# GaetanBenoitDev/metaMDBG

Hardware: AMD Instinct MI355X
Metric: Gbp/s through minimizer+k-min-mer step; bit-exact k-min-mer table vs ref (higher is better)
Workload: dtype u64

## Files before the change

### metamdbg_amd/csrc/scan.hip

```cpp
#include "common.hpp"
#include "complexity_dev.hpp"
#include "murmur.hpp"
#include "objects.hpp"
#include "prefilter.hpp"
#include "scan_plan.hpp"
#include "segments_dev.hpp"

#include <fcntl.h>
#include <sys/file.h>
#include <sys/stat.h>
#include <unistd.h>

#include <algorithm>
#include <cerrno>
#include <cmath>
#include <cstdlib>
#include <memory>
#include <mutex>
#include <string>
#include <thread>
#include <type_traits>

namespace mdbg {

// ... 497 lines not shown
                uint32_t *dst = Q->orig + cb + o;
                const uint32_t w0 = tile_base_now + lane * 32u;
#pragma unroll
                for (int half = 0; half < 2; half++) {
                    uint32_t m = half ? (uint32_t)(d >> 32) : (uint32_t)d;
                    const uint32_t wb = w0 + 16u * half;
                    while (m) {
                        *dst++ = wb + (((uint32_t)__ffs((int)m) - 1u) >> 1);
                        m &= m - 1u;
                    }
                }
            }
            wave_lds_sync();
            if (lane == 0 && cb) { atomicOr(&S[0], carry); if (HAS_N && icarry) atomicOr(&SI[0], icarry); }
            if (c) {
                unsigned dst = 2u * (cb + o), w = dst >> 5, sh = dst & 31u;
                uint32_t yl = (uint32_t)y, yh = (uint32_t)(y >> 32);
                uint32_t p0 = yl << sh;
                uint32_t p1 = sh ? ((yl >> (32u - sh)) | (yh << sh)) : yh;
                uint32_t p2 = sh ? (yh >> (32u - sh)) : 0u;
                atomicOr(&S[w], p0);
                if (p1) atomicOr(&S[w + 1], p1);
                if (p2) atomicOr(&S[w + 2], p2);
                if (HAS_N) {
                    uint32_t ic = HPC ? compress_bits(iv, d) : (iv & (nvalid == 32 ? 0xFFFFFFFFu : ((1u << nvalid) - 1u)));
                    if (ic) {
                        unsigned di = cb + o, wq = di >> 5, sq = di & 31u;
                        atomicOr(&SI[wq], ic << sq);
                        if (sq && (ic >> (32u - sq))) atomicOr(&SI[wq + 1], ic >> (32u - sq));
                    }
                }
            }
            wave_lds_sync();

            const unsigned tot = cb + C;
            const unsigned nk = tot > K ? tot - K : 0u;
            const uint32_t hp_base = hp_total - cb;
            const uint32_t tile_base = t * TILE_WORDS * 32u;
            for (unsigned j0 = 0; j0 < nk; j0 += 64 * SCAN_PP) {
                const unsigned left = nk - j0;
                const unsigned pp = left >= 64u * SCAN_PP ? (unsigned)SCAN_PP : (left + 63u) / 64u;
                KmerTrip<HPC, HAS_QUAL, HAS_N> trip{a, S, SI, Q, K, kmask, kbits, comp_mask, lane, nk, hp_base, cb, tile_base, cap0, cap, r};
                if (pp == (unsigned)SCAN_PP && left >= 64u * SCAN_PP && hp_base + j0 >= a.trim) {
                    nout = trip.template run<SCAN_PP, true>(j0, nout);
                } else {
#if SCAN_PP <= 4
                    switch (pp) {
                        case 1: nout = trip.template run<1, false>(j0, nout); break;
                        case 2: nout = trip.template run<2, false>(j0, nout); break;
                        case 3: nout = trip.template run<3, false>(j0, nout); break;
                        default: nout = trip.template run<4, false>(j0, nout); break;
                    }
#else
                    if (pp <= 2) nout = trip.template run<2, false>(j0, nout);
                    else if (pp <= 4) nout = trip.template run<4, false>(j0, nout);
                    else nout = trip.template run<SCAN_PP, false>(j0, nout);
#endif
                }
            }

            const unsigned cbn = tot < K ? tot : K;
            const uint32_t cmask = (cbn >= 16) ? 0xFFFFFFFFu : ((1u << (2 * cbn)) - 1u);
            carry = cbn ? stream_extract(S, tot - cbn, cmask) : 0u;
            if (HAS_N) icarry = cbn ? istream_extract(SI, tot - cbn, (1u << cbn) - 1u) : 0u;
            uint32_t my_orig = 0;
            if (HAS_QUAL && HPC) { if (lane < cbn) my_orig = Q->orig[tot - cbn + lane]; }
            cb = cbn;
            hp_total += C;
            wave_lds_sync();
            if (HAS_QUAL && HPC) { if (lane < cbn) Q->orig[lane] = my_orig; }
        }

        if (a.trim == 0u && hp_total >= K) {
            if (HAS_QUAL && HPC) wave_lds_sync();
            const uint32_t e = carry & kmask;
            const uint32_t rev = e ^ comp_mask, fwd = digit_reverse(e, K);
            const uint32_t d = fwd < rev ? 0u : 1u, v = d ? rev : fwd;
            bool s1 = kmer_hash32(v) < a.threshold;
            if (HAS_N) s1 = s1 && icarry == 0u;
            if (s1 && a.n_rep) s1 = !rep_contains(a.rep, a.n_rep, v);
            if (s1) {
                if (lane == 0 && nout < cap) {
                    const uint32_t p = hp_total - K;
                    a.out_min[cap0 + nout] = v;
                    a.out_pos[cap0 + nout] = p;
                    a.out_dir[cap0 + nout] = (uint8_t)d;
                    if (HAS_QUAL) {
                        const uint32_t os = HPC ? Q->orig[0] : p;
                        const uint32_t oe = a.q_last ? (HPC ? Q->orig[K - 1] : p + K - 1u) + 1u : L;
                        if (a.inline_minq) {
                            const uint8_t *qq = a.qual + a.qual_off[r];
                            uint8_t mq = 255;
                            for (uint32_t bq = os; bq < oe; bq++) { uint8_t q = (uint8_t)(qq[bq] - 33); if (q < mq) mq = q; }
                            a.out_mqual[cap0 + nout] = mq;
                        } else {
                            a.out_os[cap0 + nout] = os;
                            a.out_oe[cap0 + nout] = oe;
                        }
                    }
                }
                nout++;
            }
        }

        uint8_t flags = 0;
        if (a.apply_filters && L >= 66) {
            if (complexity_suspect(wave_sum_u64(cx_bound), complexity_windows(L))) flags |= READ_SUSPECT;
        }
        if (lane == 0) {
            a.out_count[r] = nout;
            a.out_flags[r] = flags;
        }
    }
}

constexpr int FAST_BLOCK = 256;
constexpr int FAST_WAVES = FAST_BLOCK / 64;
constexpr unsigned RING_BASES = 16384;
constexpr unsigned DEFER_BLOCKS = 3;
constexpr unsigned SPAN = 32;
constexpr unsigned BLOCK_POS = 64 * SPAN;
constexpr bool DUAL_CHAIN = true;
constexpr int STAGE_CAP = 384;

struct SpanState {
    uint32_t fwd;
    uint32_t bits;
};

template <bool APPROX, bool K15 = false>
__device__ __forceinline__ void span_step(SpanState &st, uint32_t T, bool first, uint32_t kmask, uint32_t comp_mask, unsigned top_shift,
                                          unsigned K, uint64_t threshold, uint32_t cand_limit, uint32_t Tprev = 0u) {
    const uint32_t rev = (T ^ comp_mask) & kmask;
    if (K15) st.fwd = first ? digit_reverse(T & kmask, K) : (__builtin_amdgcn_alignbit(st.fwd, Tprev, 30) & kmask);
    else st.fwd = first ? digit_reverse(T & kmask, K) : (((st.fwd << 2) | ((T >> top_shift) & 3u)) & kmask);
    const uint32_t val = st.fwd < rev ? st.fwd : rev;
    if (APPROX) {
        const uint32_t s1 = kmer_hash32_hi_merged(val);
        asm("v_cmp_lt_u32 vcc, %1, %2\n\tv_addc_co_u32 %0, vcc, %0, %0, vcc" : "+v"(st.bits) : "v"(s1), "s"(cand_limit) : "vcc");
    } else {
        const uint64_t h = kmer_hash32(val);
        asm("v_cmp_lt_u64 vcc, %1, %2\n\tv_addc_co_u32 %0, vcc, %0, %0, vcc" : "+v"(st.bits) : "v"(h), "s"(threshold) : "vcc");
    }
}

__device__ __forceinline__ uint32_t ring_window(const uint32_t *S, unsigned p, unsigned wmask) {
    const unsigned b = 2u * p, w = (b >> 5) & wmask, sh = b & 31u;
    return __builtin_amdgcn_alignbit(S[(w + 1) & wmask], S[w], sh);
}

constexpr int HIST_TILES = 8;

constexpr unsigned PF_RING_BASES = 8192;
constexpr unsigned PF_DEFER_BLOCKS = 1;
constexpr int PF_STAGE_CAP = 176;
constexpr unsigned PF_LIST_CAP = 224;
template <int PFW> struct FastGeometry {
    static constexpr bool PF = PFW > 0;
    static constexpr int WAVES = PF ? PFW : FAST_WAVES, BLOCK = 64 * WAVES, STAGE = PF ? PF_STAGE_CAP : STAGE_CAP;
    static constexpr unsigned RING = PF ? PF_RING_BASES : RING_BASES, DEFER = PF ? PF_DEFER_BLOCKS : DEFER_BLOCKS;
    static constexpr unsigned RING_WORDS = RING / 16, RING_WMASK = RING_WORDS - 1;
    static constexpr size_t PF_LDS = PREFILTER_BYTES + 2 * HPC_LUT_SIZE + REP_FILTER_BITS / 8 + 16 +
                                     (size_t)WAVES * (RING / 4 + STAGE * 8 + PF_LIST_CAP * 2 + 64 * 4);
};
static_assert(FastGeometry<16>::PF_LDS + 28672 <= 163840, "16 waves fit beside the 28 KB the benchmark's other batch asks for");

template <bool HPC, bool QUAL, bool APPROX, int PFW = 0, bool SEG = false>
__global__ __launch_bounds__(FastGeometry<PFW>::BLOCK, PFW ? PFW / 4 : 5) void scan_fast_kernel(ScanArgs a) {
    using Geo = FastGeometry<PFW>;
    constexpr bool PF = Geo::PF;
    static_assert(!PF || (HPC && !QUAL && APPROX), "the bitmap holds the keys of compressed reads; its candidates are confirmed like APPROX ones");
    static_assert(Geo::DEFER * BLOCK_POS + 2 * BLOCK_POS + 17 <= Geo::RING, "deferred blocks + live bases fit the ring");
    __shared__ uint8_t lds_stage_q[QUAL ? Geo::WAVES : 1][QUAL ? Geo::STAGE : 1];
    __shared__ uint16_t lds_hist_o[(QUAL && HPC) ? Geo::WAVES * HIST_TILES * 64 : 1];
    __shared__ uint32_t lds_hist_c[(QUAL && HPC) ? Geo::WAVES : 1][(QUAL && HPC) ? HIST_TILES : 1];
    __shared__ alignas(16) uint32_t lds_ring[Geo::WAVES][Geo::RING_WORDS];
    __shared__ uint2 lds_stage[Geo::WAVES][Geo::STAGE];
    __shared__ alignas(16) uint8_t lds_lut[HPC ? 2 * HPC_LUT_SIZE : 16];
    const uint8_t *lds_lut_b = lds_lut, *lds_lut_n = lds_lut + (HPC ? HPC_LUT_SIZE : 0);
    __shared__ alignas(16) uint32_t lds_rep_filter[REP_FILTER_BITS / 32];
    if (HPC) hpc_lut_to_lds(lds_lut, threadIdx.x, Geo::BLOCK);
    static_assert((Geo::WAVES * Geo::RING_WORDS) % (4 * Geo::BLOCK) == 0 && (REP_FILTER_BITS / 32) % 4 == 0, "cleared as uint4");
#pragma unroll
    for (unsigned i = 0; i < Geo::WAVES * Geo::RING_WORDS / 4u; i += Geo::BLOCK) reinterpret_cast<uint4 *>(&lds_ring[0][0])[i + threadIdx.x] = make_uint4(0u, 0u, 0u, 0u);
    if (threadIdx.x < REP_FILTER_BITS / 128u) reinterpret_cast<uint4 *>(lds_rep_filter)[threadIdx.x] = make_uint4(0u, 0u, 0u, 0u);
    const uint8_t *pf_map = nullptr;
    uint16_t *pf_list_all = nullptr;
    uint32_t *pf_surv_all = nullptr, *pf_next = nullptr;
    if constexpr (PF) {
        __shared__ alignas(16) uint32_t lds_pf_map[PREFILTER_BYTES / 4];
        __shared__ uint16_t lds_pf_list[Geo::WAVES][PF_LIST_CAP];
        __shared__ uint32_t lds_pf_surv[Geo::WAVES][64];
        __shared__ uint32_t lds_pf_next;
        for (unsigned i = threadIdx.x; i < PREFILTER_BYTES / 16u; i += Geo::BLOCK)
            reinterpret_cast<uint4 *>(lds_pf_map)[i] = reinterpret_cast<const uint4 *>(a.pf_bits)[i];
        if (threadIdx.x == 0) lds_pf_next = 0u;
        pf_map = reinterpret_cast<const uint8_t *>(lds_pf_map);
        pf_list_all = &lds_pf_list[0][0]; pf_surv_all = &lds_pf_surv[0][0]; pf_next = &lds_pf_next;
    }
    __syncthreads();
    for (unsigned i = threadIdx.x; i < a.n_rep; i += Geo::BLOCK) {
        const uint32_t b = rep_filter_bit(a.rep[i]);
        atomicOr(&lds_rep_filter[b >> 5], 1u << (b & 31u));
    }
    __syncthreads();
    if (a.wave_priority == 1u) __builtin_amdgcn_s_setprio(1);
    else if (a.wave_priority == 2u) __builtin_amdgcn_s_setprio(2);
    else if (a.wave_priority >= 3u) __builtin_amdgcn_s_setprio(3);
    const unsigned lane = threadIdx.x & 63u;
    const unsigned wv = (unsigned)__builtin_amdgcn_readfirstlane((int)(threadIdx.x >> 6));
    uint32_t *S = lds_ring[wv];
    uint2 *stage = lds_stage[wv];
    uint8_t *stage_q = lds_stage_q[QUAL ? wv : 0];
    uint16_t *hist_o = lds_hist_o + ((QUAL && HPC) ? wv * HIST_TILES * 64 : 0);
    uint32_t *hist_c = lds_hist_c[(QUAL && HPC) ? wv : 0];
    const unsigned K = a.K;
    const uint32_t kmask = (K >= 16) ? 0xFFFFFFFFu : ((1u << (2 * K)) - 1u);
    const uint32_t comp_mask = 0xAAAAAAAAu & kmask;
    const unsigned top_shift = 2u * K - 2u;
    const uint64_t threshold = a.threshold;
    const uint64_t cand_limit64 = (threshold >> 32) + 3ull + (uint64_t)a.cand_slack;
    const uint32_t cand_limit = cand_limit64 > 0xFFFFFFFFull ? 0xFFFFFFFFu : (uint32_t)cand_limit64;
    const uint64_t guard_limit64 = 68ull + (uint64_t)a.guard_slack;
    const uint32_t guard_limit = guard_limit64 > 0xFFFFFFFFull ? 0xFFFFFFFFu : (uint32_t)guard_limit64;
    const bool unguarded = HPC && K == 15u && a.guard_slack == 0u;

    const uint32_t wave_global = blockIdx.x * Geo::WAVES + wv;
    const uint32_t n_waves = gridDim.x * Geo::WAVES;
    uint16_t *pf_list = PF ? pf_list_all + wv * PF_LIST_CAP : nullptr;
    uint32_t *pf_surv = PF ? pf_surv_all + wv * 64u : nullptr;
    const uint32_t pf_shift = a.pf_shift;
    const uint4 *const pf_table = PF ? a.pf_table : nullptr;
    const uint32_t pf_table_shift = a.pf_table_shift;
    constexpr uint32_t NO_READ = 0xFFFFFFFFu;
    const uint64_t chunk0 = (uint64_t)blockIdx.x * a.pf_chunk;
    const uint32_t chunk_n = PF ? (chunk0 >= a.n_reads ? 0u : (uint32_t)(a.n_reads - chunk0 < a.pf_chunk ? a.n_reads - chunk0 : a.pf_chunk)) : 0u;
    unsigned long long *const pf_counter = PF ? a.pf_counter : nullptr;
    uint32_t run_next = 0, run_end = 0, run_region = 0;
    auto take_read = [&]() -> uint32_t {
        if (pf_counter) {
            if (run_next == run_end) {
                uint32_t lo = 0, hi = 0;
                if (lane == 0) {
                    const unsigned long long s0 = __hip_atomic_fetch_add(pf_counter, (unsigned long long)a.pf_grab, __ATOMIC_RELAXED, __HIP_MEMORY_SCOPE_AGENT);
                    lo = (uint32_t)s0; hi = (uint32_t)(s0 >> 32);
                }
                lo = (uint32_t)__builtin_amdgcn_readfirstlane((int)lo); hi = (uint32_t)__builtin_amdgcn_readfirstlane((int)hi);
                if (hi || lo >= a.n_reads) return NO_READ;
                run_next = lo;
                run_end = a.n_reads - lo < a.pf_grab ? a.n_reads : lo + a.pf_grab;
                run_region = (lo / a.pf_grab) & (a.n_regions - 1u);
            }
            return run_next++;
        }
        uint32_t k = 0;
        if (lane == 0) k = atomicAdd(pf_next, 1u);
        k = (uint32_t)__builtin_amdgcn_readfirstlane((int)k);
        return k < chunk_n ? (uint32_t)chunk0 + k : NO_READ;
    };
    for (uint32_t r = PF ? take_read() : wave_global; PF ? r != NO_READ : r < a.n_reads; r = PF ? take_read() : r + n_waves) {
        if constexpr (PF && !SEG) { if (a.pf_len_split && a.len[r] >= a.pf_len_split) continue; }
        if (!SEG && a.skip && a.skip[r]) {
            if (a.cursor && lane == 0) { a.out_begin[r] = 0; a.out_count[r] = 0; a.out_flags[r] = 0; }
            continue;
        }
        SegView view{};
        if constexpr (SEG) {
            view = a.views[r];
            if (view.flags & SEG_DEAD) {
                if (lane == 0) { a.out_begin[r] = 0; a.out_count[r] = 0; a.out_flags[r] = 0; a.view_cx[r] = 0ull; }
                continue;
            }
        }
        const uint32_t rd = SEG ? view.read : r;
        const bool seg_inner = SEG && !(view.flags & SEG_FIRST);
        const uint32_t L = SEG ? view.raw_len : a.len[r];
        const uint64_t w_base = a.word_off[rd] + (SEG ? (uint64_t)view.tile0 * TILE_WORDS : 0ull);
        const uint64_t *rw = a.words + w_base;
        const uint32_t trim_first = seg_inner ? 0u : a.trim;
        const uint32_t nwords = (L + 31u) / 32u;
        const uint32_t ntiles = (nwords + TILE_WORDS - 1) / TILE_WORDS;
        const bool bump = a.cursor != nullptr;
        const uint64_t cap0 = bump ? 0ull : a.cap_off[r];
        const uint32_t cap = bump ? 0u : (uint32_t)(a.cap_off[r + 1] - cap0);
        uint32_t t_done = 0;
        uint32_t fill = 0;
        bool outgrown = false;

        auto orig_of = [&](uint32_t j, bool at_end) -> uint32_t {
            if (at_end && j >= fill) return L;
            uint32_t tt = t_done - 1u;
            const uint32_t t_low = t_done > (uint32_t)HIST_TILES ? t_done - (uint32_t)HIST_TILES : 0u;
            while (tt > t_low && hist_c[tt % HIST_TILES] > j) tt--;
            const uint32_t c0 = hist_c[tt % HIST_TILES];
            if (c0 > j) return 0xFFFFFFFFu;
            const uint32_t rel = j - c0;
            const uint16_t *o = hist_o + (tt % HIST_TILES) * 64u;
            uint32_t lo = 0;
#pragma unroll
            for (uint32_t st = 16; st >= 1; st >>= 2) {
                const uint32_t o1 = o[lo + st], o2 = o[lo + 2 * st], o3 = o[lo + 3 * st];
                lo += st * ((o1 <= rel ? 1u : 0u) + (o2 <= rel ? 1u : 0u) + (o3 <= rel ? 1u : 0u));
            }
            uint32_t k = rel - o[lo];
            const uint32_t wi = tt * TILE_WORDS + lo;
            const uint64_t x = rw[wi];
            const uint32_t pl = (wi || seg_inner) ? (uint32_t)(rw[(int64_t)wi - 1] >> 62) : (((uint32_t)x & 3u) ^ 1u);
            const int rem = (int)L - (int)(wi * 32u);
            const unsigned nvalid = rem >= 32 ? 32u : (unsigned)rem;
            const uint64_t vspread = nvalid == 32 ? M5 : (((1ull << (2 * nvalid)) - 1ull) & M5);
            const uint64_t diff = x ^ ((x << 2) | (uint64_t)pl);
            uint64_t m = (diff | (diff >> 1)) & vspread;
            uint32_t pos = 0;
#pragma unroll
            for (int sh = 32; sh >= 2; sh >>= 1) {
                const uint32_t c = (uint32_t)__popcll(m & ((1ull << sh) - 1ull));
                if (k >= c) { k -= c; m >>= sh; pos += (uint32_t)sh; }
            }
            return wi * 32u + (pos >> 1);
        };
        const uint8_t *qq = QUAL ? a.qual + a.qual_off[rd] + (SEG ? (uint64_t)view.tile0 * SEG_TILE_BASES : 0ull) : nullptr;
        auto min_quality = [&](uint32_t j, bool &known) -> uint8_t {
            uint32_t os = j, oe = j + K;
            if (HPC) {
                os = orig_of(j, false);
                const uint32_t last = orig_of(j + K - a.q_last, true);
                if (os == 0xFFFFFFFFu || last == 0xFFFFFFFFu) { known = false; return 0; }
                oe = last + a.q_last;
            }
            uint8_t mq = 255;
            for (uint32_t b0 = os; b0 < oe; b0 += 16) {
                uint64_t w[2];
                __builtin_memcpy(w, qq + b0, 16);
                const uint32_t nb = oe - b0 < 16u ? oe - b0 : 16u;
#pragma unroll
                for (unsigned b = 0; b < 16; b++) {
                    const uint8_t q = (uint8_t)((uint8_t)(w[b >> 3] >> (8 * (b & 7))) - 33);
                    if (b < nb && q < mq) mq = q;
                }
            }
            return mq;
        };

        bool lost = false;
        uint32_t n_false = 0;
        uint32_t n_staged_at_outgrowth = 0;
        uint32_t done = 0;
        uint32_t nout = 0;
        uint32_t flushed = 0;
        uint32_t n_mat = 0;
        uint32_t zero_from = 0;
        uint32_t prev_last = seg_inner ? (uint32_t)(rw[-1] >> 62) : 0u;
        static_assert((uint64_t)CX_Q_MAX * ((1ull << 24) / 16u) < (1ull << 32), "the 32-bit sum of a read below 2^24 bases");
        uint32_t cx_acc = 0;
        uint64_t cx_total = 0;
        const bool cx_long = L >= (1u << 24);
        uint64_t prev_word = seg_inner ? rw[-1] : 0ull;
        const uint32_t cx_nW = complexity_windows(SEG ? a.len[rd] : L);
        const uint32_t cx_tiles = SEG ? ((view.flags & SEG_LAST) ? ntiles : a.seg_tiles) : ntiles;
        const uint32_t cx_t0 = SEG ? view.tile0 : 0u;

        auto materialise = [&]() {
            const uint32_t pend = nout - n_mat;
            if (pend == 0u) return;
            if (outgrown) { n_mat = nout; return; }
            const uint32_t base = n_mat - flushed;
            for (uint32_t i = lane; i < pend; i += 64) {
                const uint32_t j = stage[base + i].y;
                const uint32_t e = ring_window(S, j, Geo::RING_WMASK) & kmask;
                const uint32_t rev = e ^ comp_mask, fw = digit_reverse(e, K);
                const uint32_t d = fw < rev ? 0u : 1u;
                if (QUAL) { bool known = true; stage_q[base + i] = min_quality(j, known); if (!known) lost = true; }
                stage[base + i] = make_uint2(d ? rev : fw, (j << 1) | d);
            }
            n_mat = nout;
            wave_lds_sync();
        };
        auto release_ring = [&](uint32_t upto) {
            const unsigned zb = zero_from >> 4, nz = (upto - zero_from) >> 4;
            for (unsigned i = lane; i < nz; i += 64) S[(zb + i) & Geo::RING_WMASK] = 0;
            zero_from = upto;
        };

        auto emit = [&](uint32_t bits, unsigned P, uint32_t npos_limit) {
            if constexpr (!PF) {
                if (P < 32u) bits &= (1u << P) - 1u;
                const uint32_t first_j = lane * P;
                if (first_j >= npos_limit) bits = 0;
                else if (first_j + P > npos_limit) bits &= ~((1u << (first_j + P - npos_limit)) - 1u);
                if (done == 0u && lane == 0u && trim_first) bits &= ~(1u << (P - 1u));
            }
            if (__ballot(bits != 0u) == 0ull) return;
            if (a.n_rep) {
                uint32_t b2 = bits;
                while (b2) {
                    const unsigned bit = 31u - (unsigned)__clz((int)b2);
                    b2 &= ~(1u << bit);
                    const unsigned u = P - 1u - bit;
                    const uint32_t e = ring_window(S, done + lane * P + u, Geo::RING_WMASK) & kmask;
                    const uint32_t rev = e ^ comp_mask, fw = digit_reverse(e, K);
                    const uint32_t v = fw < rev ? fw : rev, fb = rep_filter_bit(v);
                    if (((lds_rep_filter[fb >> 5] >> (fb & 31u)) & 1u) && rep_contains(a.rep, a.n_rep, v)) bits &= ~(1u << bit);
                }
            }
            const unsigned cnt = (unsigned)__popc(bits);
            const unsigned incl = wave_inclusive_sum_dpp(cnt);
            const unsigned total = (unsigned)__builtin_amdgcn_readlane((int)incl, 63);
            if (total == 0u) return;
            if (bump) {
                if (outgrown || nout + total > (unsigned)Geo::STAGE) {
                    if (!outgrown) { materialise(); n_staged_at_outgrowth = nout; }
                    if (APPROX && !PF) {
                        uint32_t bad = 0;
                        while (bits) {
                            const unsigned bit = 31u - (unsigned)__clz((int)bits);
                            bits &= ~(1u << bit);
                            const uint32_t e = ring_window(S, done + lane * P + (P - 1u - bit), Geo::RING_WMASK) & kmask;
                            const uint32_t rev = e ^ comp_mask, fw = digit_reverse(e, K);
                            if (!(kmer_hash32(fw < rev ? fw : rev) < threshold)) bad++;
                        }
                        n_false += (uint32_t)wave_sum_u64(bad);
                    }
                    outgrown = true; nout += total; return;
                }
            } else if (nout - flushed + total > (unsigned)Geo::STAGE) {
                materialise();
                const uint32_t ns = nout - flushed;
                for (uint32_t i = lane; i < ns; i += 64) {
                    const uint32_t idx = flushed + i;
                    if (idx < cap) {
                        const uint2 e = stage[i];
                        a.out_min[cap0 + idx] = e.x; a.out_pos[cap0 + idx] = e.y >> 1; a.out_dir[cap0 + idx] = (uint8_t)(e.y & 1u);
                        if (QUAL) a.out_mqual[cap0 + idx] = stage_q[i];
                    }
                }
                flushed = nout;
                wave_lds_sync();
            }
            if (total <= (unsigned)Geo::STAGE) {
                uint32_t at = nout - flushed + incl - cnt;
                while (bits) {
                    const unsigned bit = 31u - (unsigned)__clz((int)bits);
                    bits &= ~(1u << bit);
                    stage[at++].y = done + lane * P + (P - 1u - bit);
                }
                wave_lds_sync();
            } else {
                uint32_t at = nout + incl - cnt;
                while (bits) {
                    const unsigned bit = 31u - (unsigned)__clz((int)bits);
                    bits &= ~(1u << bit);
                    const unsigned u = P - 1u - bit;
                    const uint32_t j = done + lane * P + u;
                    const uint32_t e = ring_window(S, j, Geo::RING_WMASK) & kmask;
                    const uint32_t rev = e ^ comp_mask, fw = digit_reverse(e, K);
                    const uint32_t d = fw < rev ? 0u : 1u;
                    if (at < cap) {
                        a.out_min[cap0 + at] = d ? rev : fw; a.out_pos[cap0 + at] = j; a.out_dir[cap0 + at] = (uint8_t)d;
                        if (QUAL) { bool known = true; a.out_mqual[cap0 + at] = min_quality(j, known); if (!known) lost = true; }
                    }
                    at++;
                }
                flushed = nout + total;
                n_mat = nout + total;
            }
            nout += total;
        };

        auto pf_probe = [&](uint32_t v, uint32_t &b) {
            const uint32_t h = v * 0x9E3779B1u;
            const uint32_t byte = pf_map[h >> (pf_shift + 3u)];
            b = (b << 1) | ((byte >> ((h >> pf_shift) & 7u)) & 1u);
        };
        auto confirm = [&](uint32_t bits, unsigned P, uint32_t npos_limit) -> uint32_t {
            if (P < 32u) bits &= (1u << P) - 1u;
            {
                const uint32_t first_j = lane * P;
                if (first_j >= npos_limit) bits = 0;
                else if (first_j + P > npos_limit) bits &= ~((1u << (first_j + P - npos_limit)) - 1u);
                if (done == 0u && lane == 0u && trim_first) bits &= ~(1u << (P - 1u));
            }
            uint32_t kept = 0u;
            unsigned cnt = (unsigned)__popc(bits);
            unsigned incl = wave_inclusive_sum_dpp(cnt);
            unsigned total = (unsigned)__builtin_amdgcn_readlane((int)incl, 63);
            while (total != 0u) {
                pf_surv[lane] = 0u;
                unsigned at = incl - cnt;
                while (bits && at < PF_LIST_CAP) {
                    const unsigned bit = 31u - (unsigned)__clz((int)bits);
                    bits &= ~(1u << bit);
                    pf_list[at++] = (uint16_t)((lane << 5) | bit);
                }
                const unsigned n = total < PF_LIST_CAP ? total : PF_LIST_CAP;
                wave_lds_sync();
                auto listed_key = [&](uint32_t q) -> uint32_t {
                    const uint32_t e = ring_window(S, done + (q >> 5) * P + (P - 1u - (q & 31u)), Geo::RING_WMASK) & kmask;
                    const uint32_t rev = e ^ comp_mask, fw = digit_reverse(e, K);
                    return fw < rev ? fw : rev;
                };
                if (pf_table != nullptr) {
                    constexpr unsigned ROUNDS = (PF_LIST_CAP + 63u) / 64u;
                    uint32_t lh[ROUNDS];
                    uint4 lw[ROUNDS];
#pragma unroll
                    for (unsigned k = 0; k < ROUNDS; k++) {
                        lh[k] = 0u; lw[k] = make_uint4(0u, 0u, 0u, 0u);
                        if (64u * k < n) {
                            const unsigned i = lane + 64u * k;
                            if (i < n) {
                                lh[k] = confirm_hash(listed_key(pf_list[i]));
                                lw[k] = pf_table[lh[k] >> pf_table_shift];
                            }
                        }
                    }
                    uint32_t ask = 0u;
#pragma unroll
                    for (unsigned k = 0; k < ROUNDS; k++) {
                        if (64u * k < n) {
                            const uint32_t verdict = confirm_verdict(lw[k].x, lw[k].y, lw[k].z, lw[k].w, lh[k]);
                            if (verdict == CONFIRM_YES) { const uint32_t q = pf_list[lane + 64u * k]; atomicOr(&pf_surv[q >> 5], 1u << (q & 31u)); }
                            if (verdict == CONFIRM_ASK) ask |= 1u << k;
                        }
                    }
                    if (__ballot(ask != 0u) != 0ull) {
#pragma nounroll
                        for (unsigned k = 0; k < ROUNDS; k++) {
                            if ((ask >> k) & 1u) {
                                const uint32_t q = pf_list[lane + 64u * k];
                                if (kmer_hash32(listed_key(q)) < threshold) atomicOr(&pf_surv[q >> 5], 1u << (q & 31u));
                            }
                        }
                    }
                } else {
                    for (unsigned i = lane; i < n; i += 64u) {
                        const uint32_t q = pf_list[i];
                        if (kmer_hash32(listed_key(q)) < threshold) atomicOr(&pf_surv[q >> 5], 1u << (q & 31u));
                    }
                }
                wave_lds_sync();
                kept |= pf_surv[lane];
                if (total <= PF_LIST_CAP) break;
                wave_lds_sync();
                cnt = (unsigned)__popc(bits);
                incl = wave_inclusive_sum_dpp(cnt);
                total -= PF_LIST_CAP;
            }
            return kept;
        };

        auto guarded_redo = [&](unsigned P) -> uint32_t {
            SpanState rs{0u, 0u};
#pragma nounroll
            for (unsigned u = 0; u < P; u++)
                span_step<APPROX>(rs, ring_window(S, done + lane * P + u, Geo::RING_WMASK), u == 0u, kmask, comp_mask, top_shift, K, threshold, cand_limit);
            return rs.bits;
        };

        auto aligned_block = [&](auto sp_tag) {
            constexpr int SP = decltype(sp_tag)::value;
            constexpr unsigned WPL = (unsigned)SP / 16u;
            const unsigned wb = ((done >> 4) + WPL * lane) & Geo::RING_WMASK;
            const uint32_t W0 = S[wb], W1 = S[(wb + 1) & Geo::RING_WMASK], W2 = SP > 16 ? S[(wb + 2) & Geo::RING_WMASK] : 0u;
            SpanState st{0u, 0u};
            auto walk = [&](auto k15_tag, auto guard_tag) {
                constexpr bool K15 = decltype(k15_tag)::value;
                constexpr bool GUARD = APPROX && decltype(guard_tag)::value;
                if (SP == 32 && DUAL_CHAIN) {
                    uint32_t fa = 0u, fb = 0u, ba = 0u, bb = 0u, pa = 0u, pb = 0u;
                    uint32_t g = 0xFFFFFFFFu;
#pragma unroll
                    for (int u = 0; u < 16; u++) {
                        const uint32_t Ta = u == 0 ? W0 : __builtin_amdgcn_alignbit(W1, W0, 2 * u);
                        const uint32_t Tb = u == 0 ? W1 : __builtin_amdgcn_alignbit(W2, W1, 2 * u);
                        const uint32_t reva = (Ta ^ comp_mask) & kmask, revb = (Tb ^ comp_mask) & kmask;
                        if (u == 0) { fa = digit_reverse(Ta & kmask, K); fb = digit_reverse(Tb & kmask, K); }
                        else if (K15) { fa = __builtin_amdgcn_alignbit(fa, pa, 30) & kmask; fb = __builtin_amdgcn_alignbit(fb, pb, 30) & kmask; }
                        else { fa = ((fa << 2) | ((Ta >> top_shift) & 3u)) & kmask; fb = ((fb << 2) | ((Tb >> top_shift) & 3u)) & kmask; }
                        const uint32_t va = fa < reva ? fa : reva, vb = fb < revb ? fb : revb;
                        if (PF) {
                            pf_probe(va, ba); pf_probe(vb, bb);
                        } else if (APPROX) {
                            uint32_t ra, rb;
                            kmer_hash32_hi_shared_x2<GUARD>(va, vb, ra, rb, g);
                            asm("v_cmp_lt_u32 vcc, %1, %2\n\tv_addc_co_u32 %0, vcc, %0, %0, vcc" : "+v"(ba) : "v"(ra), "s"(cand_limit) : "vcc");
                            asm("v_cmp_lt_u32 vcc, %1, %2\n\tv_addc_co_u32 %0, vcc, %0, %0, vcc" : "+v"(bb) : "v"(rb), "s"(cand_limit) : "vcc");
                        } else {
                            const uint64_t ha = kmer_hash32(va), hb = kmer_hash32(vb);
                            asm("v_cmp_lt_u64 vcc, %1, %2\n\tv_addc_co_u32 %0, vcc, %0, %0, vcc" : "+v"(ba) : "v"(ha), "s"(threshold) : "vcc");
                            asm("v_cmp_lt_u64 vcc, %1, %2\n\tv_addc_co_u32 %0, vcc, %0, %0, vcc" : "+v"(bb) : "v"(hb), "s"(threshold) : "vcc");
                        }
                        pa = Ta; pb = Tb;
                    }
                    st.bits = (ba << 16) | bb;
                    if (GUARD && __ballot(g < guard_limit) != 0ull) {
                        if (g < guard_limit) st.bits = guarded_redo(32u);
                    }
                    return;
                }
                uint32_t Tprev = 0u;
#pragma unroll
                for (int u = 0; u < SP; u++) {
                    const uint32_t T = u == 0 ? W0 : (u < 16 ? __builtin_amdgcn_alignbit(W1, W0, 2 * u)
                                                             : (u == 16 ? W1 : __builtin_amdgcn_alignbit(W2, W1, 2 * (u - 16))));
                    span_step<APPROX, K15>(st, T, u == 0, kmask, comp_mask, top_shift, K, threshold, cand_limit, Tprev);
                    Tprev = T;
                }
            };
            if constexpr (PF) {
                walk(std::true_type(), std::false_type());
                st.bits = confirm(st.bits, (unsigned)SP, 64u * (unsigned)SP);
            } else if (K == 15u) { if (APPROX && !unguarded) walk(std::true_type(), std::true_type()); else walk(std::true_type(), std::false_type()); }
            else walk(std::false_type(), std::integral_constant<bool, APPROX>());
            emit(st.bits, (unsigned)SP, 64u * (unsigned)SP);
            wave_lds_sync();
            done += 64u * (unsigned)SP;
            constexpr unsigned defer = (QUAL && HPC) ? Geo::DEFER - 1u : Geo::DEFER;
            if (nout - n_mat >= 48u || nout == n_mat || done - zero_from > defer * BLOCK_POS) {
                materialise();
                release_ring(done);
            }
            wave_lds_sync();
        };

        uint64_t x_next = (lane < nwords) ? rw[lane] : 0;
        for (uint32_t t = 0; t < ntiles; t++) {
            const uint64_t x = x_next;
            const uint32_t wi = t * TILE_WORDS + lane;
            {
                const uint32_t nwi = wi + TILE_WORDS;
                x_next = (nwi < nwords) ? rw[nwi] : 0;
            }
            const int rem = (int)L - (int)(wi * 32u);
            const unsigned nvalid = rem <= 0 ? 0u : (rem >= 32 ? 32u : (unsigned)rem);

            if (a.apply_filters && (!SEG || t < cx_tiles)) {
                const uint32_t xl = (uint32_t)x, xh = (uint32_t)(x >> 32);
                const uint32_t pl32 = lane_below(xl, (uint32_t)prev_word), ph32 = lane_below(xh, (uint32_t)(prev_word >> 32));
                prev_word = ((uint64_t)(uint32_t)__builtin_amdgcn_readlane((int)xh, 63) << 32) | (uint32_t)__builtin_amdgcn_readlane((int)xl, 63);
                const uint32_t q = word_pair_q(((uint64_t)ph32 << 32) | pl32, xl);
                const uint32_t tg = t + cx_t0;
                if (tg != 0u && tg * TILE_WORDS + (TILE_WORDS - 1u) <= cx_nW) {
                    cx_acc += q + q;
                } else {
                    const uint32_t wq = cx_t0 * TILE_WORDS + wi - 1u;
                    const uint32_t w2 = wq < cx_nW ? q : 0u, w1 = (wq - 1u) < cx_nW ? q : 0u;
                    cx_acc += w2 + w1;
                }
                if (cx_long) { cx_total += wave_sum_u32(cx_acc); cx_acc = 0; }
            }

            uint64_t y;
            unsigned c;
            if (HPC) {
                uint32_t pl = lane_below((uint32_t)(x >> 62), prev_last);
                if (wi == 0 && !seg_inner) pl = ((uint32_t)x & 3u) ^ 1u;
                unsigned nbits;
                y = compress_pairs_lut(HpcLut{lds_lut_b, lds_lut_n}, x, pl, &nbits);
                c = nbits >> 1;
                if (nvalid < 32) {
                    const uint64_t vspread = ((1ull << (2 * nvalid)) - 1ull) & M5;
                    const uint64_t diff = x ^ ((x << 2) | (uint64_t)pl);
                    const uint64_t d = (diff | (diff >> 1)) & vspread;
                    c = (unsigned)__popcll(d);
                    y &= c >= 32 ? ~0ull : ((1ull << (2 * c)) - 1ull);
                }
                prev_last = (uint32_t)__builtin_amdgcn_readlane((int)(uint32_t)(x >> 62), 63);
            } else {
                c = nvalid;
                y = nvalid == 32 ? x : (x & ((1ull << (2 * nvalid)) - 1ull));
            }
            const unsigned inc = wave_inclusive_sum_dpp(c);
            const unsigned o = inc - c;
            const unsigned C = (unsigned)__builtin_amdgcn_readlane((int)inc, 63);

            if (c) {
                const unsigned dst = 2u * ((fill + o) & (Geo::RING - 1u)), w = dst >> 5, sh = dst & 31u;
                const uint32_t yl = (uint32_t)y, yh = (uint32_t)(y >> 32);
                const uint32_t p0 = yl << sh;
                const uint32_t p1 = sh ? ((yl >> (32u - sh)) | (yh << sh)) : yh;
                const uint32_t p2 = sh ? (yh >> (32u - sh)) : 0u;
                atomicOr(&S[w], p0);
                if (p1) atomicOr(&S[(w + 1) & Geo::RING_WMASK], p1);
                if (p2) atomicOr(&S[(w + 2) & Geo::RING_WMASK], p2);
            }
            if (HPC && QUAL) {
                hist_o[(t % HIST_TILES) * 64u + lane] = (uint16_t)o;
                if (lane == 0) hist_c[t % HIST_TILES] = fill;
                t_done = t + 1u;
            }
            fill += C;
            wave_lds_sync();

            while (fill - done >= BLOCK_POS + K + a.trim && (!SEG || view.n_own - done >= BLOCK_POS)) aligned_block(std::integral_constant<int, (int)SPAN>());
        }

        {
            const uint32_t live = fill - done;
            uint32_t npos = live > K ? live - K : 0u;
            if (a.trim == 0u && live >= K) npos = live - K + 1u;
            if (SEG && npos > view.n_own - done) npos = view.n_own - done;
            npos = (uint32_t)__builtin_amdgcn_readfirstlane((int)npos);
            if (npos) {
                if (npos > BLOCK_POS) __builtin_trap();
                const unsigned P = (npos + 63u) >> 6;
                const unsigned Ph = (P + 1u) >> 1;
                auto chain_words = [&](unsigned p, uint32_t &lo, uint32_t &hi) {
                    const unsigned b = 2u * p, w = (b >> 5) & Geo::RING_WMASK, sh = b & 31u;
                    const uint32_t w0 = S[w], w1 = S[(w + 1) & Geo::RING_WMASK], w2 = S[(w + 2) & Geo::RING_WMASK];
                    lo = __builtin_amdgcn_alignbit(w1, w0, sh); hi = __builtin_amdgcn_alignbit(w2, w1, sh);
                };
                uint32_t bits = 0u;
                auto tail_walk = [&](auto k15_tag, auto guard_tag) {
                    constexpr bool K15 = decltype(k15_tag)::value;
                    constexpr bool GUARD = APPROX && decltype(guard_tag)::value;
                    uint32_t A0, A1, B0, B1;
                    chain_words(done + lane * P, A0, A1);
                    chain_words(done + lane * P + Ph, B0, B1);
                    uint32_t Ta = A0, Tb = B0;
                    uint32_t fa = digit_reverse(Ta & kmask, K), fb = digit_reverse(Tb & kmask, K);
                    uint32_t ba = 0u, bb = 0u;
                    uint32_t g = 0xFFFFFFFFu;
                    unsigned u = 0u;
#pragma nounroll
                    do {
                        const uint32_t reva = (Ta ^ comp_mask) & kmask, revb = (Tb ^ comp_mask) & kmask;
                        const uint32_t va = fa < reva ? fa : reva, vb = fb < revb ? fb : revb;
                        if (PF) {
                            pf_probe(va, ba); pf_probe(vb, bb);
                        } else if (APPROX) {
                            uint32_t ra, rb;
                            kmer_hash32_hi_shared_x2<GUARD>(va, vb, ra, rb, g);
                            asm("v_cmp_lt_u32 vcc, %1, %2\n\tv_addc_co_u32 %0, vcc, %0, %0, vcc" : "+v"(ba) : "v"(ra), "s"(cand_limit) : "vcc");
                            asm("v_cmp_lt_u32 vcc, %1, %2\n\tv_addc_co_u32 %0, vcc, %0, %0, vcc" : "+v"(bb) : "v"(rb), "s"(cand_limit) : "vcc");
                        } else {
                            const uint64_t ha = kmer_hash32(va), hb = kmer_hash32(vb);
                            asm("v_cmp_lt_u64 vcc, %1, %2\n\tv_addc_co_u32 %0, vcc, %0, %0, vcc" : "+v"(ba) : "v"(ha), "s"(threshold) : "vcc");
                            asm("v_cmp_lt_u64 vcc, %1, %2\n\tv_addc_co_u32 %0, vcc, %0, %0, vcc" : "+v"(bb) : "v"(hb), "s"(threshold) : "vcc");
                        }
                        u++;
                        const uint32_t Na = __builtin_amdgcn_alignbit(A1, A0, 2u * u), Nb = __builtin_amdgcn_alignbit(B1, B0, 2u * u);
                        if (K15) { fa = __builtin_amdgcn_alignbit(fa, Ta, 30) & kmask; fb = __builtin_amdgcn_alignbit(fb, Tb, 30) & kmask; }
                        else { fa = ((fa << 2) | ((Na >> top_shift) & 3u)) & kmask; fb = ((fb << 2) | ((Nb >> top_shift) & 3u)) & kmask; }
                        Ta = Na; Tb = Nb;
                    } while (u < Ph);
                    bits = (ba << (P - Ph)) | (bb >> (2u * Ph - P));
                    if (GUARD && __ballot(g < guard_limit) != 0ull) {
                        if (g < guard_limit) bits = guarded_redo(P);
                    }
                };
                if constexpr (PF) {
                    tail_walk(std::true_type(), std::false_type());
                    bits = confirm(bits, P, npos);
                } else if (K == 15u) { if (APPROX && !unguarded) tail_walk(std::true_type(), std::true_type()); else tail_walk(std::true_type(), std::false_type()); }
                else tail_walk(std::false_type(), std::integral_constant<bool, APPROX>());
                emit(bits, P, npos);
            }
            wave_lds_sync();
            materialise();
            release_ring(((fill + 15u) & ~15u) + 16u);
        }

        if (APPROX && !PF) {
            const uint32_t n_staged = outgrown ? n_staged_at_outgrowth : nout;
            for (uint32_t i = lane; i < ((n_staged + 63u) & ~63u); i += 64) {
                const uint64_t fb = __ballot(i < n_staged && !(kmer_hash32(stage[i].x) < threshold));
                if (fb) { n_false += (uint32_t)__popcll(fb); lost = true; }
            }
        }
        if (((QUAL && HPC) || (APPROX && !PF)) && __ballot(lost) != 0ull) outgrown = true;
        uint8_t flags = 0;
        if constexpr (SEG) {
            const uint64_t cx_view = a.apply_filters ? cx_total + wave_sum_u32(cx_acc) : 0ull;
            if (lane == 0) a.view_cx[r] = cx_view;
        } else if (a.apply_filters && L >= 66) {
            if (complexity_suspect(cx_total + wave_sum_u32(cx_acc), cx_nW)) flags |= READ_SUSPECT;
        }
        if (bump) {
            uint64_t start = 0;
            if (!outgrown && nout) {
                uint32_t lo = 0, hi = 0;
                const uint32_t region = pf_counter ? run_region : wave_global & (a.n_regions - 1u);
                if (lane == 0) { const unsigned long long s0 = atomicAdd(a.cursor + region, (unsigned long long)nout); lo = (uint32_t)s0; hi = (uint32_t)(s0 >> 32); }
                start = ((uint64_t)(uint32_t)__builtin_amdgcn_readfirstlane((int)hi) << 32) | (uint32_t)__builtin_amdgcn_readfirstlane((int)lo);
                const bool fits = start + nout <= a.out_capacity;
                start += (uint64_t)region * a.out_capacity;
                if (fits) {
                    for (uint32_t i = lane; i < nout; i += 64) {
                        const uint2 e = stage[i];
                        a.out_min[start + i] = e.x; a.out_pos[start + i] = e.y >> 1; a.out_dir[start + i] = (uint8_t)(e.y & 1u);
                        if (QUAL) a.out_mqual[start + i] = stage_q[i];
                    }
                }
            }
            if (lane == 0) {
                a.out_begin[r] = start;
                a.out_count[r] = nout - n_false;
                a.out_flags[r] = flags;
                if (outgrown) a.over_list[atomicAdd(&a.list_counters[0], 1u)] = r;
                if (flags & READ_SUSPECT) a.suspect_list[atomicAdd(&a.list_counters[1], 1u)] = r;
            }
        } else {
            const uint32_t ns = nout - flushed;
            for (uint32_t i = lane; i < ns; i += 64) {
                const uint32_t idx = flushed + i;
                if (idx < cap) {
                    const uint2 e = stage[i];
                    a.out_min[cap0 + idx] = e.x; a.out_pos[cap0 + idx] = e.y >> 1; a.out_dir[cap0 + idx] = (uint8_t)(e.y & 1u);
                    if (QUAL) a.out_mqual[cap0 + idx] = stage_q[i];
                }
            }
            if (lane == 0) {
                a.out_count[r] = nout;
                a.out_flags[r] = flags;
            }
        }
        wave_lds_sync();
    }
}

__global__ __launch_bounds__(256) void prefilter_build_kernel(uint32_t *bitmap, uint64_t threshold, unsigned log2_bits, uint32_t *n_set) {
    prefilter_build_range(blockIdx.x * 256u + threadIdx.x, gridDim.x * 256u, threshold, log2_bits, [&](uint32_t idx) {
        const uint32_t bit = 1u << (idx & 31u);
        if (!(atomicOr(&bitmap[idx >> 5], bit) & bit)) atomicAdd(n_set, 1u);
    });
}

struct ConfirmAtomicOps {
    __device__ uint32_t add(uint32_t *p, uint32_t v) const { return atomicAdd(p, v); }
    __device__ uint32_t orr(uint32_t *p, uint32_t v) const { return atomicOr(p, v); }
};
__global__ __launch_bounds__(256) void confirm_table_insert_kernel(uint32_t *table, uint32_t *counts, uint64_t threshold, unsigned log2_buckets) {
    confirm_table_insert_range(blockIdx.x * 256u + threadIdx.x, gridDim.x * 256u, threshold, log2_buckets, table, counts, ConfirmAtomicOps());
}
__global__ __launch_bounds__(256) void confirm_table_finish_kernel(uint32_t *table, const uint32_t *counts, unsigned log2_buckets, uint32_t *n_over) {
    for (uint32_t b = blockIdx.x * 256u + threadIdx.x; b < (1u << log2_buckets); b += gridDim.x * 256u)
        if (confirm_table_finish_bucket(table + (size_t)b * CONFIRM_BUCKET_WORDS, counts[b])) atomicAdd(n_over, 1u);
}
__global__ __launch_bounds__(256) void confirm_table_verify_kernel(uint32_t *table, uint64_t threshold, unsigned log2_buckets, uint32_t *n_over) {
    confirm_table_verify_range(blockIdx.x * 256u + threadIdx.x, gridDim.x * 256u, threshold, log2_buckets, table, ConfirmAtomicOps(),
                               [&]() { atomicAdd(n_over, 1u); });
}

__global__ __launch_bounds__(256) void split_skip_kernel(const uint32_t *len, const uint8_t *masked, uint32_t n_reads, uint32_t limit, uint8_t *skip,
                                                         unsigned long long *long_bases) {
    uint64_t sum = 0;
    for (uint64_t i = (uint64_t)blockIdx.x * 256u + threadIdx.x; i < n_reads; i += (uint64_t)gridDim.x * 256u) {
        const uint32_t L = len[i];
        skip[i] = (uint8_t)((L < limit || (masked && masked[i])) ? 1u : 0u);
        if (L >= limit) sum += L;
    }
    sum = wave_sum_u64(sum);
    if ((threadIdx.x & 63u) == 0u && sum) atomicAdd(long_bases, (unsigned long long)sum);
}

__global__ __launch_bounds__(256) void seg_count_kernel(const uint32_t *len, const uint8_t *masked, uint32_t n_reads, uint32_t G,
                                                        uint32_t *tiles_per_read, uint32_t *views_per_read, uint8_t *skip) {
    for (uint64_t i = (uint64_t)blockIdx.x * 256u + threadIdx.x; i < n_reads; i += (uint64_t)gridDim.x * 256u) {
        const uint32_t L = len[i];
        const bool plain = !(masked && masked[i]);
        const bool cut = plain && L > G;
        tiles_per_read[i] = cut ? seg_tiles(L) : 0u;
        views_per_read[i] = cut ? seg_count(L, G) : 0u;
        skip[i] = (uint8_t)(plain ? 0u : 1u);
    }
}

__global__ __launch_bounds__(256) void seg_tile_runs_kernel(const uint64_t *words, const uint64_t *word_off, const uint32_t *len, uint32_t n_reads,
                                                            const uint64_t *tile_off , uint32_t *tile_runs) {
    const unsigned lane = threadIdx.x & 63u;
    const uint64_t n_tiles = tile_off[n_reads];
    for (uint64_t gt = ((uint64_t)blockIdx.x * 256u + threadIdx.x) >> 6; gt < n_tiles; gt += ((uint64_t)gridDim.x * 256u) >> 6) {
        uint32_t lo = 0, hi = n_reads;
        while (hi - lo > 1u) { const uint32_t mid = lo + (hi - lo) / 2u; if (tile_off[mid] <= gt) lo = mid; else hi = mid; }
        const uint32_t r = lo, L = len[r], t = (uint32_t)(gt - tile_off[r]);
        const uint64_t *rw = words + word_off[r];
        const uint32_t nwords = (uint32_t)(((uint64_t)L + 31u) / 32u), wi = t * 64u + lane;
        uint32_t c = 0;
        if (wi < nwords) {
            const uint32_t prev = wi ? (uint32_t)(rw[wi - 1u] >> 62) : seg_first_prev(rw[0]);
            c = seg_word_run_starts(rw[wi], prev, seg_word_valid(L, wi));
        }
        c = (uint32_t)__builtin_amdgcn_readlane((int)wave_inclusive_sum_dpp(c), 63);
        if (lane == 0) tile_runs[gt] = c;
    }
}

__global__ __launch_bounds__(256) void seg_plan_kernel(const uint32_t *len, uint32_t n_reads, uint32_t G, uint32_t K, int hpc, const uint64_t *tile_off,
                                                       const uint64_t *view_off, const uint32_t *tile_runs, uint32_t *tile_excl ,
                                                       SegView *views, uint8_t *skip, uint8_t *read_cut, unsigned long long *totals) {
    const unsigned lane = threadIdx.x & 63u;
    for (uint64_t r = ((uint64_t)blockIdx.x * 256u + threadIdx.x) >> 6; r < n_reads; r += ((uint64_t)gridDim.x * 256u) >> 6) {
        const uint32_t nS = (uint32_t)(view_off[r + 1] - view_off[r]);
        if (nS == 0u) { if (lane == 0) read_cut[r] = 0; continue; }
        const uint32_t L = len[r], nT = (uint32_t)(tile_off[r + 1] - tile_off[r]), per = G / SEG_TILE_BASES;
        const uint32_t *tr = tile_runs + tile_off[r];
        uint32_t *te = tile_excl + tile_off[r];
        bool bad = false;
        uint32_t C = L;
        if (hpc) {
            for (uint32_t s = 1u + lane; s < nS; s += 64u) bad = bad || !seg_cut_ok(L, s * G, tr[(uint64_t)s * per], K);
            uint32_t carry = 0;
            for (uint32_t t0 = 0; t0 < nT; t0 += 64u) {
                const uint32_t t = t0 + lane, c = t < nT ? tr[t] : 0u;
                const uint32_t inc = wave_inclusive_sum_dpp(c);
                if (t < nT) te[t] = carry + inc - c;
                carry += (uint32_t)__builtin_amdgcn_readlane((int)inc, 63);
            }
            C = carry;
            __threadfence();
        } else {
            for (uint32_t s = 1u + lane; s < nS; s += 64u) {
// ... 1010 lines not shown
```

Before: 1453.

## Stage prefilter-confirmed k-mers directly instead of via survivor bitmask and re-walk

In the prefilter path, confirm now computes each listed k-mer's canonical value and position once and appends confirmed survivors straight into the stage buffer with a ballot/mbcnt compaction. This replaces the LDS survivor bitmask, its atomics, and the later emit/materialise pass that re-read the ring. Because staging is now immediate, the ring no longer needs a deferred block, and the per-wave survivor array is removed from the LDS budget. It also adds a register clobber hint and forces bump-mode staging for the PF path, which changes the output ordering and capacity handling.

```diff
diff --git a/metamdbg_amd/csrc/scan.hip b/metamdbg_amd/csrc/scan.hip
--- a/metamdbg_amd/csrc/scan.hip
+++ b/metamdbg_amd/csrc/scan.hip
@@ -673,7 +673,7 @@
 constexpr int HIST_TILES = 8;
 
 constexpr unsigned PF_RING_BASES = 8192;
-constexpr unsigned PF_DEFER_BLOCKS = 1;
+constexpr unsigned PF_DEFER_BLOCKS = 0;
 constexpr int PF_STAGE_CAP = 176;
 constexpr unsigned PF_LIST_CAP = 224;
 template <int PFW> struct FastGeometry {
@@ -682,7 +682,7 @@
     static constexpr unsigned RING = PF ? PF_RING_BASES : RING_BASES, DEFER = PF ? PF_DEFER_BLOCKS : DEFER_BLOCKS;
     static constexpr unsigned RING_WORDS = RING / 16, RING_WMASK = RING_WORDS - 1;
     static constexpr size_t PF_LDS = PREFILTER_BYTES + 2 * HPC_LUT_SIZE + REP_FILTER_BITS / 8 + 16 +
-                                     (size_t)WAVES * (RING / 4 + STAGE * 8 + PF_LIST_CAP * 2 + 64 * 4);
+                                     (size_t)WAVES * (RING / 4 + STAGE * 8 + PF_LIST_CAP * 2);
 };
 static_assert(FastGeometry<16>::PF_LDS + 28672 <= 163840, "16 waves fit beside the 28 KB the benchmark's other batch asks for");
 
@@ -692,6 +692,7 @@
     constexpr bool PF = Geo::PF;
     static_assert(!PF || (HPC && !QUAL && APPROX), "the bitmap holds the keys of compressed reads; its candidates are confirmed like APPROX ones");
     static_assert(Geo::DEFER * BLOCK_POS + 2 * BLOCK_POS + 17 <= Geo::RING, "deferred blocks + live bases fit the ring");
+    if constexpr (PF) asm volatile("" ::: "v103");
     __shared__ uint8_t lds_stage_q[QUAL ? Geo::WAVES : 1][QUAL ? Geo::STAGE : 1];
     __shared__ uint16_t lds_hist_o[(QUAL && HPC) ? Geo::WAVES * HIST_TILES * 64 : 1];
     __shared__ uint32_t lds_hist_c[(QUAL && HPC) ? Geo::WAVES : 1][(QUAL && HPC) ? HIST_TILES : 1];
@@ -707,17 +708,16 @@
     if (threadIdx.x < REP_FILTER_BITS / 128u) reinterpret_cast<uint4 *>(lds_rep_filter)[threadIdx.x] = make_uint4(0u, 0u, 0u, 0u);
     const uint8_t *pf_map = nullptr;
     uint16_t *pf_list_all = nullptr;
-    uint32_t *pf_surv_all = nullptr, *pf_next = nullptr;
+    uint32_t *pf_next = nullptr;
     if constexpr (PF) {
         __shared__ alignas(16) uint32_t lds_pf_map[PREFILTER_BYTES / 4];
         __shared__ uint16_t lds_pf_list[Geo::WAVES][PF_LIST_CAP];
-        __shared__ uint32_t lds_pf_surv[Geo::WAVES][64];
         __shared__ uint32_t lds_pf_next;
         for (unsigned i = threadIdx.x; i < PREFILTER_BYTES / 16u; i += Geo::BLOCK)
             reinterpret_cast<uint4 *>(lds_pf_map)[i] = reinterpret_cast<const uint4 *>(a.pf_bits)[i];
         if (threadIdx.x == 0) lds_pf_next = 0u;
         pf_map = reinterpret_cast<const uint8_t *>(lds_pf_map);
-        pf_list_all = &lds_pf_list[0][0]; pf_surv_all = &lds_pf_surv[0][0]; pf_next = &lds_pf_next;
+        pf_list_all = &lds_pf_list[0][0]; pf_next = &lds_pf_next;
     }
     __syncthreads();
     for (unsigned i = threadIdx.x; i < a.n_rep; i += Geo::BLOCK) {
@@ -749,7 +749,6 @@
     const uint32_t wave_global = blockIdx.x * Geo::WAVES + wv;
     const uint32_t n_waves = gridDim.x * Geo::WAVES;
     uint16_t *pf_list = PF ? pf_list_all + wv * PF_LIST_CAP : nullptr;
-    uint32_t *pf_surv = PF ? pf_surv_all + wv * 64u : nullptr;
     const uint32_t pf_shift = a.pf_shift;
     const uint4 *const pf_table = PF ? a.pf_table : nullptr;
     const uint32_t pf_table_shift = a.pf_table_shift;
@@ -801,7 +800,7 @@
         const uint32_t trim_first = seg_inner ? 0u : a.trim;
         const uint32_t nwords = (L + 31u) / 32u;
         const uint32_t ntiles = (nwords + TILE_WORDS - 1) / TILE_WORDS;
-        const bool bump = a.cursor != nullptr;
+        const bool bump = PF || a.cursor != nullptr;
         const uint64_t cap0 = bump ? 0ull : a.cap_off[r];
         const uint32_t cap = bump ? 0u : (uint32_t)(a.cap_off[r + 1] - cap0);
         uint32_t t_done = 0;
@@ -904,7 +903,7 @@
         };
 
         auto emit = [&](uint32_t bits, unsigned P, uint32_t npos_limit) {
-            if constexpr (!PF) {
+            {
                 if (P < 32u) bits &= (1u << P) - 1u;
                 const uint32_t first_j = lane * P;
                 if (first_j >= npos_limit) bits = 0;
@@ -931,7 +930,7 @@
             if (bump) {
                 if (outgrown || nout + total > (unsigned)Geo::STAGE) {
                     if (!outgrown) { materialise(); n_staged_at_outgrowth = nout; }
-                    if (APPROX && !PF) {
+                    if (APPROX) {
                         uint32_t bad = 0;
                         while (bits) {
                             const unsigned bit = 31u - (unsigned)__clz((int)bits);
@@ -993,7 +992,7 @@
             const uint32_t byte = pf_map[h >> (pf_shift + 3u)];
             b = (b << 1) | ((byte >> ((h >> pf_shift) & 7u)) & 1u);
         };
-        auto confirm = [&](uint32_t bits, unsigned P, uint32_t npos_limit) -> uint32_t {
+        auto confirm = [&](uint32_t bits, unsigned P, uint32_t npos_limit) {
             if (P < 32u) bits &= (1u << P) - 1u;
             {
                 const uint32_t first_j = lane * P;
@@ -1001,12 +1000,30 @@
                 else if (first_j + P > npos_limit) bits &= ~((1u << (first_j + P - npos_limit)) - 1u);
                 if (done == 0u && lane == 0u && trim_first) bits &= ~(1u << (P - 1u));
             }
-            uint32_t kept = 0u;
+            auto listed_row = [&](uint32_t q, uint32_t &v, uint32_t &y) {
+                const uint32_t j = done + (q >> 5) * P + (P - 1u - (q & 31u));
+                const uint32_t e = ring_window(S, j, Geo::RING_WMASK) & kmask;
+                const uint32_t rev = e ^ comp_mask, fw = digit_reverse(e, K);
+                const uint32_t d = fw < rev ? 0u : 1u;
+                v = d ? rev : fw; y = (j << 1) | d;
+            };
+            auto repetitive = [&](uint32_t v) -> bool {
+                const uint32_t fb = rep_filter_bit(v);
+                return ((lds_rep_filter[fb >> 5] >> (fb & 31u)) & 1u) && rep_contains(a.rep, a.n_rep, v);
+            };
+            auto stage_round = [&](bool sel, uint32_t v, uint32_t y) {
+                if (a.n_rep) { if (sel && repetitive(v)) sel = false; }
+                const uint64_t m = __ballot(sel);
+                if (m == 0ull) return;
+                const unsigned c = (unsigned)__popcll(m);
+                if (outgrown || nout + c > (unsigned)Geo::STAGE) outgrown = true;
+                else if (sel) stage[nout - flushed + __builtin_amdgcn_mbcnt_hi((uint32_t)(m >> 32), __builtin_amdgcn_mbcnt_lo((uint32_t)m, 0u))] = make_uint2(v, y);
+                nout += c;
+            };
             unsigned cnt = (unsigned)__popc(bits);
             unsigned incl = wave_inclusive_sum_dpp(cnt);
             unsigned total = (unsigned)__builtin_amdgcn_readlane((int)incl, 63);
             while (total != 0u) {
-                pf_surv[lane] = 0u;
                 unsigned at = incl - cnt;
                 while (bits && at < PF_LIST_CAP) {
                     const unsigned bit = 31u - (unsigned)__clz((int)bits);
@@ -1015,59 +1032,49 @@
                 }
                 const unsigned n = total < PF_LIST_CAP ? total : PF_LIST_CAP;
                 wave_lds_sync();
-                auto listed_key = [&](uint32_t q) -> uint32_t {
-                    const uint32_t e = ring_window(S, done + (q >> 5) * P + (P - 1u - (q & 31u)), Geo::RING_WMASK) & kmask;
-                    const uint32_t rev = e ^ comp_mask, fw = digit_reverse(e, K);
-                    return fw < rev ? fw : rev;
-                };
                 if (pf_table != nullptr) {
                     constexpr unsigned ROUNDS = (PF_LIST_CAP + 63u) / 64u;
-                    uint32_t lh[ROUNDS];
+                    uint32_t lv[ROUNDS], ly[ROUNDS];
                     uint4 lw[ROUNDS];
 #pragma unroll
                     for (unsigned k = 0; k < ROUNDS; k++) {
-                        lh[k] = 0u; lw[k] = make_uint4(0u, 0u, 0u, 0u);
+                        lv[k] = 0u; ly[k] = 0u; lw[k] = make_uint4(0u, 0u, 0u, 0u);
                         if (64u * k < n) {
                             const unsigned i = lane + 64u * k;
                             if (i < n) {
-                                lh[k] = confirm_hash(listed_key(pf_list[i]));
-                                lw[k] = pf_table[lh[k] >> pf_table_shift];
+                                listed_row(pf_list[i], lv[k], ly[k]);
+                                lw[k] = pf_table[confirm_hash(lv[k]) >> pf_table_shift];
                             }
                         }
                     }
-                    uint32_t ask = 0u;
 #pragma unroll
                     for (unsigned k = 0; k < ROUNDS; k++) {
                         if (64u * k < n) {
-                            const uint32_t verdict = confirm_verdict(lw[k].x, lw[k].y, lw[k].z, lw[k].w, lh[k]);
-                            if (verdict == CONFIRM_YES) { const uint32_t q = pf_list[lane + 64u * k]; atomicOr(&pf_surv[q >> 5], 1u << (q & 31u)); }
-                            if (verdict == CONFIRM_ASK) ask |= 1u << k;
-                        }
-                    }
-                    if (__ballot(ask != 0u) != 0ull) {
-#pragma nounroll
-                        for (unsigned k = 0; k < ROUNDS; k++) {
-                            if ((ask >> k) & 1u) {
-                                const uint32_t q = pf_list[lane + 64u * k];
-                                if (kmer_hash32(listed_key(q)) < threshold) atomicOr(&pf_surv[q >> 5], 1u << (q & 31u));
+                            const uint32_t verdict = confirm_verdict(lw[k].x, lw[k].y, lw[k].z, lw[k].w, confirm_hash(lv[k]));
+                            bool sel = verdict == CONFIRM_YES;
+                            if (__ballot(verdict == CONFIRM_ASK) != 0ull) {
+                                if (verdict == CONFIRM_ASK) sel = kmer_hash32(lv[k]) < threshold;
                             }
+                            stage_round(sel, lv[k], ly[k]);
                         }
                     }
                 } else {
-                    for (unsigned i = lane; i < n; i += 64u) {
-                        const uint32_t q = pf_list[i];
-                        if (kmer_hash32(listed_key(q)) < threshold) atomicOr(&pf_surv[q >> 5], 1u << (q & 31u));
+                    for (unsigned i0 = 0u; i0 < n; i0 += 64u) {
+                        uint32_t v = 0u, y = 0u;
+                        bool sel = false;
+                        if (i0 + lane < n) {
+                            listed_row(pf_list[i0 + lane], v, y);
+                            sel = kmer_hash32(v) < threshold;
+                        }
+                        stage_round(sel, v, y);
                     }
                 }
-                wave_lds_sync();
-                kept |= pf_surv[lane];
                 if (total <= PF_LIST_CAP) break;
                 wave_lds_sync();
                 cnt = (unsigned)__popc(bits);
                 incl = wave_inclusive_sum_dpp(cnt);
                 total -= PF_LIST_CAP;
             }
-            return kept;
         };
 
         auto guarded_redo = [&](unsigned P) -> uint32_t {
@@ -1130,18 +1137,24 @@
             };
             if constexpr (PF) {
                 walk(std::true_type(), std::false_type());
-                st.bits = confirm(st.bits, (unsigned)SP, 64u * (unsigned)SP);
-            } else if (K == 15u) { if (APPROX && !unguarded) walk(std::true_type(), std::true_type()); else walk(std::true_type(), std::false_type()); }
-            else walk(std::false_type(), std::integral_constant<bool, APPROX>());
-            emit(st.bits, (unsigned)SP, 64u * (unsigned)SP);
-            wave_lds_sync();
-            done += 64u * (unsigned)SP;
-            constexpr unsigned defer = (QUAL && HPC) ? Geo::DEFER - 1u : Geo::DEFER;
-            if (nout - n_mat >= 48u || nout == n_mat || done - zero_from > defer * BLOCK_POS) {
-                materialise();
+                confirm(st.bits, (unsigned)SP, 64u * (unsigned)SP);
+                wave_lds_sync();
+                done += 64u * (unsigned)SP;
                 release_ring(done);
-            }
-            wave_lds_sync();
+                wave_lds_sync();
+            } else {
+                if (K == 15u) { if (APPROX && !unguarded) walk(std::true_type(), std::true_type()); else walk(std::true_type(), std::false_type()); }
+                else walk(std::false_type(), std::integral_constant<bool, APPROX>());
+                emit(st.bits, (unsigned)SP, 64u * (unsigned)SP);
+                wave_lds_sync();
+                done += 64u * (unsigned)SP;
+                constexpr unsigned defer = (QUAL && HPC) ? Geo::DEFER - 1u : Geo::DEFER;
+                if (nout - n_mat >= 48u || nout == n_mat || done - zero_from > defer * BLOCK_POS) {
+                    materialise();
+                    release_ring(done);
+                }
+                wave_lds_sync();
+            }
         };
 
         uint64_t x_next = (lane < nwords) ? rw[lane] : 0;
@@ -1272,13 +1285,13 @@
                 };
                 if constexpr (PF) {
                     tail_walk(std::true_type(), std::false_type());
-                    bits = confirm(bits, P, npos);
+                    confirm(bits, P, npos);
                 } else if (K == 15u) { if (APPROX && !unguarded) tail_walk(std::true_type(), std::true_type()); else tail_walk(std::true_type(), std::false_type()); }
                 else tail_walk(std::false_type(), std::integral_constant<bool, APPROX>());
-                emit(bits, P, npos);
+                if constexpr (!PF) emit(bits, P, npos);
             }
             wave_lds_sync();
-            materialise();
+            if constexpr (!PF) materialise();
             release_ring(((fill + 15u) & ~15u) + 16u);
         }
 
```

Measured after the change: 1500 (median of 6 runs). 1.03x the previous value.
